# cmp-nct/ggllm.cpp

Hardware: NVIDIA B200
Metric: falcon40b_q4_k_decode_tokens_per_s (higher is better)
Workload: dtype int8 x int4 block dots (dp4a), fp32 accumulate; f32 KV/attention

## Files before the change

### ggllm.cpp_b200/csrc/common.cuh

```cuda
#pragma once
#include <cuda_runtime.h>
#include <cuda_fp16.h>
#include <cstdint>
#include <cstdio>
#include <cstdlib>

#define B200_CUDA_CHECK(expr)                                                                        \
    do {                                                                                             \
        cudaError_t err_ = (expr);                                                                   \
        if (err_ != cudaSuccess) {                                                                   \
            fprintf(stderr, "b200: CUDA error %d (%s) at %s:%d: %s\n", (int) err_,                   \
                    cudaGetErrorString(err_), __FILE__, __LINE__, #expr);                            \
            exit(1);                                                                                 \
        }                                                                                            \
    } while (0)

#define B200_ASSERT(x)                                                                               \
    do {                                                                                             \
        if (!(x)) {                                                                                  \
            fprintf(stderr, "B200_ASSERT: %s:%d: %s\n", __FILE__, __LINE__, #x);                     \
            abort();                                                                                 \
        }                                                                                            \
    } while (0)

enum : int {
    T_F32 = 0, T_F16 = 1, T_Q4_0 = 2, T_Q4_1 = 3, T_Q5_0 = 6, T_Q5_1 = 7, T_Q8_0 = 8, T_Q8_1 = 9,
    T_Q2_K = 10, T_Q3_K = 11, T_Q4_K = 12, T_Q5_K = 13, T_Q6_K = 14, T_Q8_K = 15,
};

static inline size_t round_up(size_t v, size_t a) { return (v + a - 1) / a * a; }

#define B200_CARVEOUT 25

#ifdef __CUDACC__

__device__ __forceinline__ uint4 ldg_stream_v4(const void * p) {
    uint4 r;
    asm volatile("ld.global.nc.L1::no_allocate.v4.u32 {%0,%1,%2,%3}, [%4];"
                 : "=r"(r.x), "=r"(r.y), "=r"(r.z), "=r"(r.w) : "l"(p));
    return r;
}
__device__ __forceinline__ uint2 ldg_stream_v2(const void * p) {
    uint2 r;
    asm volatile("ld.global.nc.L1::no_allocate.v2.u32 {%0,%1}, [%2];" : "=r"(r.x), "=r"(r.y) : "l"(p));
    return r;
}
__device__ __forceinline__ uint32_t ldg_stream_u32(const void * p) {
    uint32_t r;
    asm volatile("ld.global.nc.L1::no_allocate.u32 %0, [%1];" : "=r"(r) : "l"(p));
    return r;
}
__device__ __forceinline__ uint4 ldg_v4(const void * p) { return __ldg(reinterpret_cast<const uint4 *>(p)); }
__device__ __forceinline__ uint32_t ldg_u32(const void * p) { return __ldg(reinterpret_cast<const uint32_t *>(p)); }
__device__ __forceinline__ uint16_t ldg_u16(const void * p) { return __ldg(reinterpret_cast<const uint16_t *>(p)); }

__device__ __forceinline__ float f16_bits_to_f32(uint16_t h) { return __half2float(__ushort_as_half(h)); }
__device__ __forceinline__ uint16_t f32_to_f16_bits(float f) { return __half_as_ushort(__float2half_rn(f)); }

__device__ __forceinline__ float warp_sum(float v) {
#pragma unroll
    for (int o = 16; o > 0; o >>= 1) v += __shfl_xor_sync(0xffffffffu, v, o);
    return v;
}
__device__ __forceinline__ float warp_max(float v) {
#pragma unroll
    for (int o = 16; o > 0; o >>= 1) v = fmaxf(v, __shfl_xor_sync(0xffffffffu, v, o));
    return v;
}
__device__ __forceinline__ double warp_sum_d(double v) {
#pragma unroll
    for (int o = 16; o > 0; o >>= 1) v += __shfl_xor_sync(0xffffffffu, v, o);
    return v;
}

__device__ __forceinline__ int dp4a_ss(int a, int b, int c) { return __dp4a(a, b, c); }
__device__ __forceinline__ int dp4a_us(unsigned a, int b, int c) {
    int d;
    asm("dp4a.u32.s32 %0, %1, %2, %3;" : "=r"(d) : "r"(a), "r"(b), "r"(c));
    return d;
}

__device__ __forceinline__ uint32_t smem_u32(const void * p) { return (uint32_t) __cvta_generic_to_shared(p); }
__device__ __forceinline__ void mbar_init(uint64_t * bar, uint32_t count) {
    asm volatile("mbarrier.init.shared::cta.b64 [%0], %1;" :: "r"(smem_u32(bar)), "r"(count));
}
__device__ __forceinline__ void mbar_fence_init() { asm volatile("fence.mbarrier_init.release.cluster;" ::: "memory"); }
__device__ __forceinline__ void mbar_expect_tx(uint64_t * bar, uint32_t bytes) {
    asm volatile("mbarrier.arrive.expect_tx.shared::cta.b64 _, [%0], %1;" :: "r"(smem_u32(bar)), "r"(bytes) : "memory");
}
__device__ __forceinline__ void mbar_wait(uint64_t * bar, uint32_t phase) {
    asm volatile(
        "{\n\t.reg .pred p;\n\t"
        "WAIT_%=:\n\t"
        "mbarrier.try_wait.parity.shared::cta.b64 p, [%0], %1;\n\t"
        "@p bra DONE_%=;\n\t"
        "bra WAIT_%=;\n\t"
        "DONE_%=:\n\t}"
        :: "r"(smem_u32(bar)), "r"(phase) : "memory");
}
__device__ __forceinline__ void tma_load_1d(void * smem_dst, const void * gmem_src, uint32_t bytes, uint64_t * bar) {
    asm volatile("cp.async.bulk.shared::cluster.global.mbarrier::complete_tx::bytes [%0], [%1], %2, [%3];"
                 :: "r"(smem_u32(smem_dst)), "l"(gmem_src), "r"(bytes), "r"(smem_u32(bar)) : "memory");
}

__device__ __forceinline__ unsigned long long gtimer() { unsigned long long t; asm volatile("mov.u64 %0, %globaltimer;" : "=l"(t)); return t; }
__device__ __forceinline__ void trace_begin(unsigned long long * slot) { if (slot && threadIdx.x == 0) atomicMin(slot, gtimer()); }
__device__ __forceinline__ void trace_end(unsigned long long * slot) { if (slot && threadIdx.x == 0) atomicMax(slot + 1, gtimer()); }

#endif

unsigned long long * b200_trace_slot(const char * name);
```

### ggllm.cpp_b200/csrc/mmv_fast.cu

```cuda
#include "kernels.h"

#include "mmv_fast.cuh"

template <int TYPE, int NT, int J, int D, int MODE>
__device__ __forceinline__ void mmv_body(const WPlanes & W, const FastX & X, float * __restrict__ y, int64_t y_stride, const Epi & epi,
                                         const int cta, const int nctas, const int n, uint8_t * smem) {
    using T = FX<TYPE>;
    constexpr int NW = NT / 32;
    uint64_t * bar = reinterpret_cast<uint64_t *>(smem);
    float * partial = reinterpret_cast<float *>(smem + 16);
    double * red = reinterpret_cast<double *>(smem + 16 + 2 * NW * 4 * 4);
    int8_t * xq = reinterpret_cast<int8_t *>(smem + ((16 + 2 * NW * 4 * 4 + NW * 8 + 15) & ~15));
    const int tid = threadIdx.x, lane = tid & 31, warp = tid >> 5;
    const int P = W.nb * T::PPB;
    const ActQ & A = X.A;

    trace_begin(epi.trace);
    if (tid == 0 && MODE == 0) { mbar_init(bar, 1); mbar_fence_init(); }
    const int per = W.M / nctas, rem = W.M % nctas;
    const int row0 = cta * per + min(cta, rem), row1 = row0 + per + (cta < rem ? 1 : 0);
    const int nrows = row1 - row0;

    int gidx[J]; bool valid[J];
    WP wp[J];
    int aux[J];
#pragma unroll
    for (int j = 0; j < J; j++) { const int g = j * NT + tid; valid[j] = g < P; gidx[j] = valid[j] ? g : P - 1; wp[j] = T::wp(W, gidx[j]); aux[j] = piece_aux<TYPE>(gidx[j]); }

    typename T::WR w[D][J];
    ring_fill<TYPE, J, D>(w, wp, row0, row1);
    const L2PF pf = l2pf_of(W, X.l2_dist);
    if (pf.dist > 0 && tid == 0) l2_prefetch_rows(pf, min(row0 + D, row1), min(row0 + D + pf.dist, row1));

    if (!epi.late_wait) asm volatile("griddepcontrol.wait;" ::: "memory");
    typename T::XR xr[J];
    if (MODE == 0) {
        if (tid == 0) {
            mbar_expect_tx(bar, (uint32_t) W.K);
            tma_load_1d(xq, A.q + (size_t) n * W.K, (uint32_t) W.K, bar);
        }
        __syncthreads();
        mbar_wait(bar, 0);
#pragma unroll
        for (int j = 0; j < J; j++) xr[j] = valid[j] ? T::load_x(xq, A, n, gidx[j]) : zero_xr<TYPE>();
    } else if constexpr (T::HAS_PROLOGUE_QUANT) {
        const float * xrow = X.x + (size_t) n * X.x_stride;
        float mean = 0.f, scale = 1.f;
#pragma unroll
        for (int j = 0; j < J; j++) {
            int ea, eb; T::seg(gidx[j], ea, eb);
            float v[32];
#pragma unroll
            for (int i = 0; i < 4; i++) {
                const float4 a = *reinterpret_cast<const float4 *>(xrow + ea + 4 * i), b = *reinterpret_cast<const float4 *>(xrow + eb + 4 * i);
                v[4 * i] = a.x; v[4 * i + 1] = a.y; v[4 * i + 2] = a.z; v[4 * i + 3] = a.w;
                v[16 + 4 * i] = b.x; v[17 + 4 * i] = b.y; v[18 + 4 * i] = b.z; v[19 + 4 * i] = b.w;
            }
            if (MODE == 2 && J == 1) {
                if (X.ra) {
                    const float * ra = X.ra + (size_t) n * X.x_stride, * rb = X.rb + (size_t) n * X.x_stride;
#pragma unroll
                    for (int i = 0; i < 16; i++) { v[i] = __fadd_rn(__fadd_rn(ra[ea + i], rb[ea + i]), v[i]); v[16 + i] = __fadd_rn(__fadd_rn(ra[eb + i], rb[eb + i]), v[16 + i]); }
                }
                if (X.x_out && cta == 0 && valid[j]) {
                    float * xo = X.x_out + (size_t) n * X.x_stride;
#pragma unroll
                    for (int i = 0; i < 16; i++) { xo[ea + i] = v[i]; xo[eb + i] = v[16 + i]; }
                }
                double s = 0.0;
                if (valid[j]) {
#pragma unroll
                    for (int i = 0; i < 32; i++) s += (double) v[i];
                }
                s = warp_sum_d(s);
                if (lane == 0) red[warp] = s;
                __syncthreads();
                double t = 0.0;
#pragma unroll
                for (int wi = 0; wi < NW; wi++) t += red[wi];
                mean = (float) (t / W.K);
                __syncthreads();
                double s2 = 0.0;
                if (valid[j]) {
#pragma unroll
                    for (int i = 0; i < 32; i++) { const float c = __fsub_rn(v[i], mean); s2 += (double) __fmul_rn(c, c); }
                }
                s2 = warp_sum_d(s2);
                if (lane == 0) red[warp] = s2;
                __syncthreads();
                t = 0.0;
#pragma unroll
                for (int wi = 0; wi < NW; wi++) t += red[wi];
                scale = __fdiv_rn(1.0f, __fsqrt_rn(__fadd_rn((float) (t / W.K), 1e-5f)));
#pragma unroll
                for (int i = 0; i < 16; i++) {
                    v[i] = __fadd_rn(__fmul_rn(__fmul_rn(__fsub_rn(v[i], mean), scale), X.gamma[ea + i]), X.beta[ea + i]);
                    v[16 + i] = __fadd_rn(__fmul_rn(__fmul_rn(__fsub_rn(v[16 + i], mean), scale), X.gamma[eb + i]), X.beta[eb + i]);
                }
            }
            if (!valid[j]) {
#pragma unroll
                for (int i = 0; i < 32; i++) v[i] = 0.f;
            }
            xr[j] = T::quant_x(v, gidx[j], lane);
        }
        __syncthreads();
    }

    int gcount = 0;
    const int ekind = epi.kind; const float * r1p = epi.r1, * r2p = epi.r2;
    ring_run<TYPE, NT, J, D, false>(w, wp, row0, row1, wp, 0, 0, xr, aux, partial, gcount, 0, tid,
        [&](int row, float v) {
            if (ekind == EPI_GELU) v = gelu_lut(v);
            else if (ekind == EPI_ADD2) v = (v + r1p[(size_t) n * y_stride + row]) + r2p[(size_t) n * y_stride + row];
            y[(size_t) n * y_stride + row] = v;
        },
        [&]() { asm volatile("griddepcontrol.launch_dependents;" ::: "memory"); }, pf);
    if (epi.late_wait) asm volatile("griddepcontrol.wait;" ::: "memory");
    if (epi.qctr) {
        __shared__ int s_do;
        __threadfence();
        __syncthreads();
        if (nrows > 0) {
            for (int b = row0 >> 8; b <= (row1 - 1) >> 8; b++) {
                if (tid == 0) {
                    const unsigned cnt = (unsigned) (min(row1, (b + 1) << 8) - max(row0, b << 8));
                    const unsigned old = atomicAdd(epi.qctr + b, cnt);
                    s_do = old + cnt == 256u;
                    if (s_do) epi.qctr[b] = 0;
                }
                __syncthreads();
                if (s_do && warp == 0) {
                    __threadfence();
                    const float * src = y + (size_t) n * y_stride + (b << 8) + lane * 8;
                    const float4 p = __ldcg(reinterpret_cast<const float4 *>(src)), q = __ldcg(reinterpret_cast<const float4 *>(src) + 1);
                    const float v[8] = { p.x, p.y, p.z, p.w, q.x, q.y, q.z, q.w };
                    if (epi.qA.type == T_Q8_K) quantize_chunk8<T_Q8_K>(v, lane, epi.qA, n, (b << 8) + lane * 8);
                    else quantize_chunk8<T_Q8_0>(v, lane, epi.qA, n, (b << 8) + lane * 8);
                }
                __syncthreads();
            }
        }
    }
    trace_end(epi.trace);
}

template <int TYPE, int NT, int J, int D, int MODE>
__global__ void __launch_bounds__(NT) __maxnreg__(NT <= 256 ? 96 : 128) mmv_fast_kernel(const WPlanes W, const FastX X, float * __restrict__ y, int64_t y_stride, const Epi epi) {
    extern __shared__ __align__(16) uint8_t smem[];
    mmv_body<TYPE, NT, J, D, MODE>(W, X, y, y_stride, epi, (int) blockIdx.x, (int) gridDim.x, (int) blockIdx.y, smem);
}

static int fast_num_sms() {
    static int n = 0;
    if (!n) { int dev; B200_CUDA_CHECK(cudaGetDevice(&dev)); B200_CUDA_CHECK(cudaDeviceGetAttribute(&n, cudaDevAttrMultiProcessorCount, dev)); }
    return n;
}

template <int TYPE, int NT, int J, int D, int MODE>
static void launch_mode(const WPlanes & W, const FastX & X, float * y, int64_t y_stride, Epi epi, cudaStream_t stream) {
    const size_t smem = ((16 + 2 * (NT / 32) * 4 * 4 + (NT / 32) * 8 + 15) & ~15) + (size_t) ((W.K + 15) & ~15);
    static bool set = false;
    if (!set) { B200_CUDA_CHECK(cudaFuncSetAttribute(mmv_fast_kernel<TYPE, NT, J, D, MODE>, cudaFuncAttributeMaxDynamicSharedMemorySize, 100 * 1024));
        B200_CUDA_CHECK(cudaFuncSetAttribute(mmv_fast_kernel<TYPE, NT, J, D, MODE>, cudaFuncAttributePreferredSharedMemoryCarveout, B200_CARVEOUT)); set = true; }
    int ctas = fast_num_sms() * (NT == 128 ? 4 : NT == 160 || NT == 192 ? 3 : NT == 256 ? 2 : 1);
    if (ctas > (W.M + 3) / 4) ctas = (W.M + 3) / 4;
    cudaLaunchConfig_t cfg{};
    cfg.gridDim = dim3((unsigned) ctas, (unsigned) X.N); cfg.blockDim = dim3(NT); cfg.dynamicSmemBytes = smem; cfg.stream = stream;
    cudaLaunchAttribute attr[1];
    attr[0].id = cudaLaunchAttributeProgrammaticStreamSerialization;
    attr[0].val.programmaticStreamSerializationAllowed = 1;
    cfg.attrs = attr; cfg.numAttrs = getenv("B200_NO_PDL") ? 0 : 1;
    B200_CUDA_CHECK(cudaLaunchKernelEx(&cfg, mmv_fast_kernel<TYPE, NT, J, D, MODE>, W, X, y, y_stride, epi));
}
template <int TYPE, int NT, int J, int D>
static void launch_cfg(const WPlanes & W, const FastX & X, float * y, int64_t y_stride, Epi epi, cudaStream_t stream) {
    if (X.mode == 0) launch_mode<TYPE, NT, J, D, 0>(W, X, y, y_stride, epi, stream);
    else if constexpr (FX<TYPE>::HAS_PROLOGUE_QUANT) {
        if (X.mode == 1) launch_mode<TYPE, NT, J, D, 1>(W, X, y, y_stride, epi, stream);
        else if (J == 1) launch_mode<TYPE, NT, J, D, J == 1 ? 2 : 1>(W, X, y, y_stride, epi, stream);
        else B200_ASSERT(!"mmv_fast: LayerNorm prologue needs J == 1");
    } else B200_ASSERT(!"mmv_fast: this weight type takes quantised activations only (mode 0)");
}

template <int TYPE>
static bool launch_type(const WPlanes & W, const FastX & X, float * y, int64_t y_stride, Epi epi, cudaStream_t stream) {
    const int P = W.nb * FX<TYPE>::PPB;
    if (W.K > 64 * 1024) return false;
    if (X.mode == 2 && P > 512) return false;
    constexpr int D1 = FX<TYPE>::D256;
    if (P <= 128 && D1 == 4) launch_cfg<TYPE, 128, 1, D1>(W, X, y, y_stride, epi, stream);
    else if (P > 128 && P <= 160 && D1 == 8 && !getenv("B200_NO_NT160")) launch_cfg<TYPE, 160, 1, D1>(W, X, y, y_stride, epi, stream);
    else if (P <= 256) launch_cfg<TYPE, 256, 1, D1>(W, X, y, y_stride, epi, stream);
    else if (P > 256 && P <= 512 && D1 == 8 && X.mode == 0 && !getenv("B200_NO_NT256J2")) launch_cfg<TYPE, 256, 2, D1 / 2>(W, X, y, y_stride, epi, stream);
    else if (P <= 512) launch_cfg<TYPE, 512, 1, D1>(W, X, y, y_stride, epi, stream);
    else if (P > 512 && P <= 576 && D1 == 8 && X.mode == 0 && !getenv("B200_NO_NT192")) launch_cfg<TYPE, 192, 3, 2>(W, X, y, y_stride, epi, stream);
    else if (P <= 1024) launch_cfg<TYPE, 512, 2, D1 / 2>(W, X, y, y_stride, epi, stream);
    else if (P <= 2048 && D1 == 8) launch_cfg<TYPE, 512, 4, 2>(W, X, y, y_stride, epi, stream);
    else return false;
    return true;
}

bool launch_mmv_fast_x(const WPlanes & W, const FastX & X, float * y, int64_t y_stride, MmvEpilogue e, cudaStream_t stream) {
    const char * nm = W.M > 40000 ? "mmv_lmhead" : W.K > 16384 ? "mmv_down" : W.M > 16384 ? "mmv_up" : W.M > 8192 ? "mmv_qkv" : "mmv_wo";
    Epi epi = { e.kind, e.r1, e.r2, b200_trace_slot(nm), ActQ{}, nullptr, getenv("B200_NO_LATE_WAIT") ? 0 : e.late_wait };
    if (e.qout && e.qctr) {
        B200_ASSERT(X.N == 1 && W.M % 256 == 0 && e.qout->K == W.M && (e.qout->type == T_Q8_K || e.qout->type == T_Q8_0));
        epi.qA = *e.qout; epi.qctr = e.qctr;
    }
    static int dist_bytes = -1;
    if (dist_bytes < 0) { const char * s = getenv("B200_L2PF_KB"); dist_bytes = (s ? atoi(s) : 0) * 1024; }
    FastX Xp = X;
    Xp.l2_dist = W.stride[0] ? (int) (dist_bytes / W.stride[0]) : 0;
    switch (W.type) {
        case T_Q4_K: return launch_type<T_Q4_K>(W, Xp, y, y_stride, epi, stream);
        case T_Q4_0: return launch_type<T_Q4_0>(W, Xp, y, y_stride, epi, stream);
        case T_Q3_K: return X.mode == 0 && !getenv("B200_Q3K_GENERIC") && launch_type<T_Q3_K>(W, Xp, y, y_stride, epi, stream);
    }
    return false;
}
bool mmv_fast_supports(int wtype, int K, int mode) {
    if (wtype != T_Q4_K && wtype != T_Q4_0) return false;
    const int P = wtype == T_Q4_K ? K / 32 : K / 32;
    return K <= 64 * 1024 && P <= (mode == 2 ? 512 : 2048);
}
bool mmv_fast_fills_sm(const WPlanes & W) {
    if ((W.type != T_Q4_K && W.type != T_Q4_0) || getenv("B200_NO_NT192")) return false;
    const int P = W.K / 32;
    return P > 512 && P <= 576;
}
bool launch_mmv_fast(const WPlanes & W, const ActQ & A, float * y, int64_t y_stride, MmvEpilogue e, cudaStream_t stream) {
    FastX X{}; X.mode = 0; X.A = A; X.N = A.N;
    return launch_mmv_fast_x(W, X, y, y_stride, e, stream);
}
```

### ggllm.cpp_b200/csrc/mmv_fast.cuh

```cuda
#pragma once
#include "kernels.h"
#include "actquant.cuh"

struct Epi { int kind; const float * r1; const float * r2; unsigned long long * trace; ActQ qA; unsigned * qctr; int late_wait; };


__device__ __forceinline__ int dot16(const uint32_t w0, const uint32_t w1, const uint32_t w2, const uint32_t w3, const uint4 x) {
    int s = dp4a_us(w0, (int) x.x, 0); s = dp4a_us(w1, (int) x.y, s); s = dp4a_us(w2, (int) x.z, s); return dp4a_us(w3, (int) x.w, s);
}
__device__ __forceinline__ int dp2a_lo_su(int pair16, uint32_t bytes) { int d; asm("dp2a.lo.s32.u32 %0, %1, %2, %3;" : "=r"(d) : "r"(pair16), "r"(bytes), "r"(0)); return d; }
__device__ __forceinline__ int dp2a_hi_su(int pair16, uint32_t bytes) { int d; asm("dp2a.hi.s32.u32 %0, %1, %2, %3;" : "=r"(d) : "r"(pair16), "r"(bytes), "r"(0)); return d; }
__device__ __forceinline__ int dp2a_lo_ss(int pair16, uint32_t bytes, int c) { int d; asm("dp2a.lo.s32.s32 %0, %1, %2, %3;" : "=r"(d) : "r"(pair16), "r"(bytes), "r"(c)); return d; }
__device__ __forceinline__ int dp2a_hi_ss(int pair16, uint32_t bytes, int c) { int d; asm("dp2a.hi.s32.s32 %0, %1, %2, %3;" : "=r"(d) : "r"(pair16), "r"(bytes), "r"(c)); return d; }
__device__ __forceinline__ float gelu_lut(float v) {
    const float f = __half2float(__float2half_rn(v));
    const float g = 0.5f * f * (1.0f + tanhf(0.79788456080286535587989211986876f * f * (1.0f + 0.044715f * f * f)));
    return __half2float(__float2half_rn(g));
}

struct WP { const uint8_t * b0, * b1, * b2, * b3; uint32_t s0, s1, s2, s3; };
__device__ __forceinline__ const uint8_t * opaque_ptr(const uint8_t * p) { unsigned long long v = (unsigned long long) p; asm volatile("" : "+l"(v)); return (const uint8_t *) v; }

template <int TYPE> struct FX;

template <> struct FX<T_Q4_K> {
    static constexpr int PPB = 8;
    static constexpr bool HAS_PROLOGUE_QUANT = true;
    static constexpr int D256 = 8;
    struct XR { uint4 xl, xh; int bs; float xd; };
    struct WR { uint4 q; uint32_t sm, dd; };
    __device__ static XR load_x(const int8_t * xq, const ActQ & A, int n, int g) {
        const int b = g >> 3, pc = g & 7, p = pc >> 1, half = pc & 1;
        XR r;
        const int e0 = b * 256 + 64 * p + 16 * half;
        r.xl = *reinterpret_cast<const uint4 *>(xq + e0);
        r.xh = *reinterpret_cast<const uint4 *>(xq + e0 + 32);
        const int16_t * bs = A.bs + (size_t) n * (A.K / 16) + b * 16 + 4 * p + half;
        r.bs = ((int) bs[0] & 0xffff) | ((int) bs[2] << 16);
        r.xd = A.d[(size_t) n * (A.K / 256) + b];
        return r;
    }
    __device__ static void seg(int g, int & ea, int & eb) { const int b = g >> 3, pc = g & 7; ea = b * 256 + 64 * (pc >> 1) + 16 * (pc & 1); eb = ea + 32; }
    __device__ static XR quant_x(const float (&v)[32], int g, int lane) {
        int ea, eb; seg(g, ea, eb);
        float amax = 0.f, vmax = 0.f; int imax = 0;
#pragma unroll
        for (int i = 0; i < 32; i++) { const float ax = fabsf(v[i]); const int idx = (i < 16 ? ea : eb - 16) + i; if (ax > amax || (ax == amax && ax > 0.f && idx < imax)) { amax = ax; vmax = v[i]; imax = idx; } }
#pragma unroll
        for (int o = 1; o < 8; o <<= 1) {
            const float oa = __shfl_xor_sync(0xffffffffu, amax, o), ov = __shfl_xor_sync(0xffffffffu, vmax, o);
            const int oi = __shfl_xor_sync(0xffffffffu, imax, o);
            if (oa > amax || (oa == amax && oi < imax)) { amax = oa; vmax = ov; imax = oi; }
        }
        XR r;
        const bool zero = amax == 0.f;
        const float iscale = zero ? 0.f : __fdiv_rn(-128.f, vmax);
        r.xd = zero ? 0.f : __fdiv_rn(1.f, iscale);
        int s0 = 0, s1 = 0;
        uint32_t w[8];
#pragma unroll
        for (int i = 0; i < 8; i++) {
            uint32_t pk = 0;
#pragma unroll
            for (int k = 0; k < 4; k++) {
                const int q = zero ? 0 : min(127, __float2int_rn(__fmul_rn(iscale, v[4 * i + k])));
                if (i < 4) s0 += q; else s1 += q;
                pk |= (uint32_t) (q & 0xff) << (8 * k);
            }
            w[i] = pk;
        }
        r.xl = make_uint4(w[0], w[1], w[2], w[3]); r.xh = make_uint4(w[4], w[5], w[6], w[7]);
        r.bs = (s0 & 0xffff) | (s1 << 16);
        (void) lane;
        return r;
    }
    __device__ static WP wp(const WPlanes & W, int g) {
        WP r; r.b0 = opaque_ptr(W.p[0] + (size_t) g * 16); r.b1 = opaque_ptr(W.p[1] + (size_t) (g >> 1) * 4); r.b2 = opaque_ptr(W.p[2] + (size_t) (g >> 3) * 4);
        r.s0 = W.stride[0]; r.s1 = W.stride[1]; r.s2 = W.stride[2];
        return r;
    }
    __device__ static WR load_w(const WP & p, uint32_t row) {
        WR r;
        r.q = ldg_stream_v4(p.b0 + (uint64_t) row * p.s0);
        r.sm = ldg_u32(p.b1 + (uint64_t) row * p.s1);
        r.dd = ldg_u32(p.b2 + (uint64_t) row * p.s2);
        return r;
    }
    __device__ static float dot(const WR & w, const XR & x) {
        const int il = dot16(w.q.x & 0x0F0F0F0F, w.q.y & 0x0F0F0F0F, w.q.z & 0x0F0F0F0F, w.q.w & 0x0F0F0F0F, x.xl);
        const int ih = dot16(w.q.x & 0xF0F0F0F0, w.q.y & 0xF0F0F0F0, w.q.z & 0xF0F0F0F0, w.q.w & 0xF0F0F0F0, x.xh) >> 4;
        const int isum = dp2a_lo_su((il & 0xffff) | (ih << 16), w.sm);
        const int msum = dp2a_hi_su(x.bs, w.sm);
        const float2 dm = __half22float2(*reinterpret_cast<const __half2 *>(&w.dd));
        return (dm.x * x.xd) * (float) isum - (dm.y * x.xd) * (float) msum;
    }
};

template <> struct FX<T_Q4_0> {
    static constexpr int PPB = 1;
    static constexpr bool HAS_PROLOGUE_QUANT = true;
    static constexpr int D256 = 8;
    struct XR { uint4 xl, xh; int bs; float xd; };
    struct WR { uint4 q; uint32_t d; };
    __device__ static XR load_x(const int8_t * xq, const ActQ & A, int n, int g) {
        XR r;
        r.xl = *reinterpret_cast<const uint4 *>(xq + g * 32);
        r.xh = *reinterpret_cast<const uint4 *>(xq + g * 32 + 16);
        r.bs = A.bs[(size_t) n * (A.K / 32) + g];
        r.xd = A.d[(size_t) n * (A.K / 32) + g];
        return r;
    }
    __device__ static void seg(int g, int & ea, int & eb) { ea = g * 32; eb = ea + 16; }
    __device__ static XR quant_x(const float (&v)[32], int, int) {
        float amax = 0.f;
#pragma unroll
        for (int i = 0; i < 32; i++) amax = fmaxf(amax, fabsf(v[i]));
        const float id = amax != 0.f ? __fdiv_rn(127.f, amax) : 0.f;
        XR r;
        r.xd = __half2float(__float2half_rn(__fdiv_rn(amax, 127.f)));
        int s = 0;
        uint32_t w[8];
#pragma unroll
        for (int i = 0; i < 8; i++) {
            uint32_t pk = 0;
#pragma unroll
            for (int k = 0; k < 4; k++) { const int q = __float2int_rn(__fmul_rn(v[4 * i + k], id)); s += q; pk |= (uint32_t) (q & 0xff) << (8 * k); }
            w[i] = pk;
        }
        r.xl = make_uint4(w[0], w[1], w[2], w[3]); r.xh = make_uint4(w[4], w[5], w[6], w[7]);
        r.bs = s;
        return r;
    }
    __device__ static WP wp(const WPlanes & W, int g) {
        WP r; r.b0 = opaque_ptr(W.p[0] + (size_t) g * 16); r.b1 = opaque_ptr(W.p[1] + (size_t) g * 2); r.b2 = nullptr;
        r.s0 = W.stride[0]; r.s1 = W.stride[1]; r.s2 = 0;
        return r;
    }
    __device__ static WR load_w(const WP & p, uint32_t row) {
        WR r;
        r.q = ldg_stream_v4(p.b0 + (uint64_t) row * p.s0);
        r.d = ldg_u16(p.b1 + (uint64_t) row * p.s1);
        return r;
    }
    __device__ static float dot(const WR & w, const XR & x) {
        int s = dot16(w.q.x & 0x0F0F0F0F, w.q.y & 0x0F0F0F0F, w.q.z & 0x0F0F0F0F, w.q.w & 0x0F0F0F0F, x.xl);
        s += dot16(w.q.x & 0xF0F0F0F0, w.q.y & 0xF0F0F0F0, w.q.z & 0xF0F0F0F0, w.q.w & 0xF0F0F0F0, x.xh) >> 4;
        s -= 8 * x.bs;
        return ((float) s * f16_bits_to_f32((uint16_t) w.d)) * x.xd;
    }
};

template <> struct FX<T_Q3_K> {
    static constexpr int PPB = 4;
    static constexpr bool HAS_PROLOGUE_QUANT = false;
    static constexpr int D256 = 4;
    struct XR { uint4 x[4]; int bsA, bsB; float xd; };
    struct WR { uint4 q, hm; uint32_t sc, d; };
    __device__ static XR load_x(const int8_t * xq, const ActQ & A, int n, int g) {
        const int b = g >> 2, pc = g & 3, hn = pc >> 1, c = pc & 1;
        XR r;
        const int16_t * bs = A.bs + (size_t) n * (A.K / 16) + b * 16 + 8 * hn + c;
#pragma unroll
        for (int quad = 0; quad < 4; quad++) r.x[quad] = *reinterpret_cast<const uint4 *>(xq + b * 256 + 128 * hn + 32 * quad + 16 * c);
        r.bsA = ((int) bs[0] & 0xffff) | ((int) bs[2] << 16);
        r.bsB = ((int) bs[4] & 0xffff) | ((int) bs[6] << 16);
        r.xd = A.d[(size_t) n * (A.K / 256) + b];
        return r;
    }
    __device__ static void seg(int, int & ea, int & eb) { ea = 0; eb = 0; }
    __device__ static XR quant_x(const float (&)[32], int, int) { return XR{}; }
    __device__ static WP wp(const WPlanes & W, int g) {
        WP r;
        r.b0 = opaque_ptr(W.p[0] + (size_t) g * 16); r.b1 = opaque_ptr(W.p[1] + (size_t) (g >> 2) * 32 + (g & 1) * 16);
        r.b2 = opaque_ptr(W.p[2] + (size_t) g * 4);  r.b3 = opaque_ptr(W.p[3] + (size_t) (g >> 2) * 2);
        r.s0 = W.stride[0]; r.s1 = W.stride[1]; r.s2 = W.stride[2]; r.s3 = W.stride[3];
        return r;
    }
    __device__ static WR load_w(const WP & p, uint32_t row) {
        WR r;
        r.q = ldg_stream_v4(p.b0 + (uint64_t) row * p.s0);
        r.hm = ldg_v4(p.b1 + (uint64_t) row * p.s1);
        r.sc = ldg_u32(p.b2 + (uint64_t) row * p.s2);
        r.d = ldg_u16(p.b3 + (uint64_t) row * p.s3);
        return r;
    }
    __device__ static float dot(const WR & w, const XR & x, int hsh) {
        const uint32_t q[4] = { w.q.x, w.q.y, w.q.z, w.q.w }, hm[4] = { w.hm.x, w.hm.y, w.hm.z, w.hm.w };
        const uint32_t hbase = 0x01010101u << hsh;
        int i[4];
#pragma unroll
        for (int quad = 0; quad < 4; quad++) {
            const uint32_t qm = 0x03030303u << (2 * quad), hmk = hbase << quad;
            const int dq = dot16(q[0] & qm, q[1] & qm, q[2] & qm, q[3] & qm, x.x[quad]);
            const int dh = dot16(hm[0] & hmk, hm[1] & hmk, hm[2] & hmk, hm[3] & hmk, x.x[quad]);
            i[quad] = (dq >> (2 * quad)) + ((dh >> (hsh + quad)) << 2);
        }
        int isum = dp2a_lo_ss((i[0] & 0xffff) | (i[1] << 16), w.sc, 0);
        isum = dp2a_hi_ss((i[2] & 0xffff) | (i[3] << 16), w.sc, isum);
        int bsum = dp2a_lo_ss(x.bsA, w.sc, 0);
        bsum = dp2a_hi_ss(x.bsB, w.sc, bsum);
        return (f16_bits_to_f32((uint16_t) w.d) * x.xd) * (float) (isum - 4 * bsum);
    }
};

template <int G> __device__ __forceinline__ float transpose_reduce(const float (&acc)[G], int lane, int & row_of_lane) {
    float w;
    if (G == 4) {
        const bool hi = lane & 16;
        float v0 = hi ? acc[2] : acc[0], v1 = hi ? acc[3] : acc[1];
        v0 += __shfl_xor_sync(0xffffffffu, hi ? acc[0] : acc[2], 16);
        v1 += __shfl_xor_sync(0xffffffffu, hi ? acc[1] : acc[3], 16);
        const bool mid = lane & 8;
        w = mid ? v1 : v0;
        w += __shfl_xor_sync(0xffffffffu, mid ? v0 : v1, 8);
        w += __shfl_xor_sync(0xffffffffu, w, 4);
        row_of_lane = (hi ? 2 : 0) + (mid ? 1 : 0);
    } else if (G == 2) {
        const bool hi = lane & 16;
        w = hi ? acc[G - 1] : acc[0];
        w += __shfl_xor_sync(0xffffffffu, hi ? acc[0] : acc[G - 1], 16);
        w += __shfl_xor_sync(0xffffffffu, w, 8);
        w += __shfl_xor_sync(0xffffffffu, w, 4);
        row_of_lane = hi ? 1 : 0;
    } else {
        w = acc[0];
        w += __shfl_xor_sync(0xffffffffu, w, 16);
        w += __shfl_xor_sync(0xffffffffu, w, 8);
        w += __shfl_xor_sync(0xffffffffu, w, 4);
        row_of_lane = 0;
    }
    w += __shfl_xor_sync(0xffffffffu, w, 2);
    w += __shfl_xor_sync(0xffffffffu, w, 1);
    return w;
}


struct L2PF { const uint8_t * p[3]; uint32_t s[3]; int dist; };
__device__ __forceinline__ void l2_prefetch_rows(const L2PF & pf, int a, int b) {
    if (b <= a) return;
#pragma unroll
    for (int i = 0; i < 3; i++) {
        if (!pf.p[i]) continue;
        const uint8_t * src = pf.p[i] + (size_t) a * pf.s[i];
        const uint32_t bytes = (uint32_t) (b - a) * pf.s[i];
        asm volatile("cp.async.bulk.prefetch.L2.global [%0], %1;" :: "l"(src), "r"(bytes) : "memory");
    }
}
__device__ __forceinline__ L2PF l2pf_of(const WPlanes & W, int dist) {
    L2PF r; r.dist = dist;
#pragma unroll
    for (int i = 0; i < 3; i++) { r.p[i] = W.p[i]; r.s[i] = W.stride[i]; }
    return r;
}

__device__ __forceinline__ void named_sync(int id, int n) { asm volatile("bar.sync %0, %1;" :: "r"(id), "r"(n) : "memory"); }

template <int TYPE> __device__ __forceinline__ int piece_aux(int g) { return TYPE == T_Q3_K ? 4 * ((g & 3) >> 1) : 0; }
template <int TYPE> __device__ __forceinline__ float piece_dot(const typename FX<TYPE>::WR & w, const typename FX<TYPE>::XR & x, int aux) {
    if constexpr (TYPE == T_Q3_K) return FX<TYPE>::dot(w, x, aux); else return FX<TYPE>::dot(w, x);
}
template <int TYPE> __device__ __forceinline__ typename FX<TYPE>::XR zero_xr() {
    typename FX<TYPE>::XR r{}; return r;
}

template <int TYPE, int J, int D>
__device__ __forceinline__ void ring_fill(typename FX<TYPE>::WR (&w)[D][J], const WP (&wp)[J], int r0, int r1) {
    if (r1 <= r0) return;
#pragma unroll
    for (int s = 0; s < D; s++) {
        const uint32_t row = (uint32_t) min(r0 + s, r1 - 1);
#pragma unroll
        for (int j = 0; j < J; j++) w[s][j] = FX<TYPE>::load_w(wp[j], row);
    }
}

template <int TYPE, int NTG, int J, int D, bool CHECKED, bool HASNEXT, class Store>
__device__ __forceinline__ void ring_pass(typename FX<TYPE>::WR (&w)[D][J], const WP (&wp)[J], const int r0, const int nrows, const int npad, const int base,
                                          const WP (&wpn)[J], const int n0, const int n1,
                                          const typename FX<TYPE>::XR (&xr)[J], const int (&aux)[J], float * partial, int & gcount, const int bar_id, const int tg, Store & store) {
    using T = FX<TYPE>;
    constexpr int NWG = NTG / 32, G = (D % 4 == 0) ? 4 : (D % 2 == 0) ? 2 : 1;
    const int lane = tg & 31, warp = tg >> 5;
    float acc[G];
#pragma unroll
    for (int s = 0; s < D; s++) {
        float a = piece_dot<TYPE>(w[s][0], xr[0], aux[0]);
#pragma unroll
        for (int j = 1; j < J; j++) a += piece_dot<TYPE>(w[s][j], xr[j], aux[j]);
        acc[s % G] = a;
        const int nxt = base + D + s;
        if (!CHECKED || nxt < nrows) {
#pragma unroll
            for (int j = 0; j < J; j++) w[s][j] = T::load_w(wp[j], (uint32_t) (r0 + nxt));
        } else if (HASNEXT && nxt >= npad && n1 > n0) {
            const uint32_t k = (uint32_t) min(n0 + nxt - npad, n1 - 1);
#pragma unroll
            for (int j = 0; j < J; j++) w[s][j] = T::load_w(wpn[j], k);
        }
        if ((s % G) == G - 1) {
            const int gi = (base + s) / G;
            int rl;
            const float v0 = transpose_reduce<G>(acc, lane, rl);
            float * part = partial + (gcount & 1) * NWG * G;
            gcount++;
            if ((lane & (G == 4 ? 7 : G == 2 ? 15 : 31)) == 0) part[warp * G + rl] = v0;
            named_sync(bar_id, NTG);
            if (tg < G) {
                const int row = r0 + gi * G + tg;
                if (!CHECKED || row < r0 + nrows) {
                    float v = 0.f;
#pragma unroll
                    for (int wi = 0; wi < NWG; wi++) v += part[wi * G + tg];
                    store(row, v);
                }
            }
        }
    }
}

template <int TYPE, int NTG, int J, int D, bool HASNEXT, class Store, class Tail>
__device__ __forceinline__ void ring_run(typename FX<TYPE>::WR (&w)[D][J], const WP (&wp)[J], const int r0, const int r1,
                                         const WP (&wpn)[J], const int n0, const int n1,
                                         const typename FX<TYPE>::XR (&xr)[J], const int (&aux)[J], float * partial, int & gcount, const int bar_id, const int tg,
                                         Store store, Tail before_tail, const L2PF pf = L2PF{ { nullptr, nullptr, nullptr }, { 0, 0, 0 }, 0 }) {
    const int nrows = r1 - r0, npad = (nrows + D - 1) / D * D;
    if (npad == 0) { before_tail(); if (HASNEXT) ring_fill<TYPE, J, D>(w, wpn, n0, n1); return; }
    int base = 0;
    for (; base + 2 * D <= nrows; base += D) {
        if (pf.dist > 0 && tg == 0) l2_prefetch_rows(pf, min(r0 + base + D + pf.dist, r1), min(r0 + base + 2 * D + pf.dist, r1));
        ring_pass<TYPE, NTG, J, D, false, false>(w, wp, r0, nrows, npad, base, wpn, n0, n1, xr, aux, partial, gcount, bar_id, tg, store);
    }
    before_tail();
    for (; base < npad; base += D)
        ring_pass<TYPE, NTG, J, D, true, HASNEXT>(w, wp, r0, nrows, npad, base, wpn, n0, n1, xr, aux, partial, gcount, bar_id, tg, store);
}
```

Baseline: 210.2.

## Replace per-group CTA barrier with mbarrier reduction ring in matvec

Result: slower. 163.1, median of 6 (-22.4%).

```diff
diff --git a/ggllm.cpp_b200/csrc/common.cuh b/ggllm.cpp_b200/csrc/common.cuh
--- a/ggllm.cpp_b200/csrc/common.cuh
+++ b/ggllm.cpp_b200/csrc/common.cuh
@@ -81,9 +81,8 @@
 }
 
 __device__ __forceinline__ uint32_t smem_u32(const void * p) { return (uint32_t) __cvta_generic_to_shared(p); }
-__device__ __forceinline__ void mbar_init(uint64_t * bar, uint32_t count) {
-    asm volatile("mbarrier.init.shared::cta.b64 [%0], %1;" :: "r"(smem_u32(bar)), "r"(count));
-}
+__device__ __forceinline__ void mbar_init(uint32_t bar, uint32_t count) { asm volatile("mbarrier.init.shared::cta.b64 [%0], %1;" :: "r"(bar), "r"(count)); }
+__device__ __forceinline__ void mbar_init(uint64_t * bar, uint32_t count) { mbar_init(smem_u32(bar), count); }
 __device__ __forceinline__ void mbar_fence_init() { asm volatile("fence.mbarrier_init.release.cluster;" ::: "memory"); }
 __device__ __forceinline__ void mbar_expect_tx(uint64_t * bar, uint32_t bytes) {
     asm volatile("mbarrier.arrive.expect_tx.shared::cta.b64 _, [%0], %1;" :: "r"(smem_u32(bar)), "r"(bytes) : "memory");
diff --git a/ggllm.cpp_b200/csrc/mmv_fast.cu b/ggllm.cpp_b200/csrc/mmv_fast.cu
--- a/ggllm.cpp_b200/csrc/mmv_fast.cu
+++ b/ggllm.cpp_b200/csrc/mmv_fast.cu
@@ -1,22 +1,38 @@
 #include "kernels.h"
 
 #include "mmv_fast.cuh"
+
+template <int NT, int D> struct MmvSmem {
+    static constexpr int NW = NT / 32, G = ring_group<D>(), R = 4, LAG = 2;
+    using Ring = RedRing<NW, G, R>;
+    static constexpr int xbar = 0;
+    static constexpr int ring = 8;
+    static constexpr int red = (ring + Ring::BYTES + 7) & ~7;
+    static constexpr int xq = (red + NW * 8 + 15) & ~15;
+    static size_t bytes(int K) { return (size_t) xq + (size_t) ((K + 15) & ~15); }
+};
 
 template <int TYPE, int NT, int J, int D, int MODE>
 __device__ __forceinline__ void mmv_body(const WPlanes & W, const FastX & X, float * __restrict__ y, int64_t y_stride, const Epi & epi,
                                          const int cta, const int nctas, const int n, uint8_t * smem) {
     using T = FX<TYPE>;
+    using L = MmvSmem<NT, D>;
     constexpr int NW = NT / 32;
-    uint64_t * bar = reinterpret_cast<uint64_t *>(smem);
-    float * partial = reinterpret_cast<float *>(smem + 16);
-    double * red = reinterpret_cast<double *>(smem + 16 + 2 * NW * 4 * 4);
-    int8_t * xq = reinterpret_cast<int8_t *>(smem + ((16 + 2 * NW * 4 * 4 + NW * 8 + 15) & ~15));
+    uint64_t * bar = reinterpret_cast<uint64_t *>(smem + L::xbar);
+    const typename L::Ring rr = { smem_u32(smem + L::ring) };
+    double * red = reinterpret_cast<double *>(smem + L::red);
+    int8_t * xq = reinterpret_cast<int8_t *>(smem + L::xq);
     const int tid = threadIdx.x, lane = tid & 31, warp = tid >> 5;
     const int P = W.nb * T::PPB;
     const ActQ & A = X.A;
 
     trace_begin(epi.trace);
-    if (tid == 0 && MODE == 0) { mbar_init(bar, 1); mbar_fence_init(); }
+    if (tid == 0) {
+        if (MODE == 0) mbar_init(bar, 1);
+#pragma unroll
+        for (int s = 0; s < L::R; s++) { mbar_init(rr.full(s), NW * L::G); mbar_init(rr.empty(s), L::G); }
+        mbar_fence_init();
+    }
     const int per = W.M / nctas, rem = W.M % nctas;
     const int row0 = cta * per + min(cta, rem), row1 = row0 + per + (cta < rem ? 1 : 0);
     const int nrows = row1 - row0;
@@ -107,9 +123,8 @@
         __syncthreads();
     }
 
-    int gcount = 0;
     const int ekind = epi.kind; const float * r1p = epi.r1, * r2p = epi.r2;
-    ring_run<TYPE, NT, J, D, false>(w, wp, row0, row1, wp, 0, 0, xr, aux, partial, gcount, 0, tid,
+    ring_run<TYPE, NT, J, D, L::R, L::LAG>(w, wp, row0, row1, xr, aux, rr, tid,
         [&](int row, float v) {
             if (ekind == EPI_GELU) v = gelu_lut(v);
             else if (ekind == EPI_ADD2) v = (v + r1p[(size_t) n * y_stride + row]) + r2p[(size_t) n * y_stride + row];
@@ -159,7 +174,7 @@
 
 template <int TYPE, int NT, int J, int D, int MODE>
 static void launch_mode(const WPlanes & W, const FastX & X, float * y, int64_t y_stride, Epi epi, cudaStream_t stream) {
-    const size_t smem = ((16 + 2 * (NT / 32) * 4 * 4 + (NT / 32) * 8 + 15) & ~15) + (size_t) ((W.K + 15) & ~15);
+    const size_t smem = MmvSmem<NT, D>::bytes(W.K);
     static bool set = false;
     if (!set) { B200_CUDA_CHECK(cudaFuncSetAttribute(mmv_fast_kernel<TYPE, NT, J, D, MODE>, cudaFuncAttributeMaxDynamicSharedMemorySize, 100 * 1024));
         B200_CUDA_CHECK(cudaFuncSetAttribute(mmv_fast_kernel<TYPE, NT, J, D, MODE>, cudaFuncAttributePreferredSharedMemoryCarveout, B200_CARVEOUT)); set = true; }
diff --git a/ggllm.cpp_b200/csrc/mmv_fast.cuh b/ggllm.cpp_b200/csrc/mmv_fast.cuh
--- a/ggllm.cpp_b200/csrc/mmv_fast.cuh
+++ b/ggllm.cpp_b200/csrc/mmv_fast.cuh
@@ -253,8 +253,6 @@
     return r;
 }
 
-__device__ __forceinline__ void named_sync(int id, int n) { asm volatile("bar.sync %0, %1;" :: "r"(id), "r"(n) : "memory"); }
-
 template <int TYPE> __device__ __forceinline__ int piece_aux(int g) { return TYPE == T_Q3_K ? 4 * ((g & 3) >> 1) : 0; }
 template <int TYPE> __device__ __forceinline__ float piece_dot(const typename FX<TYPE>::WR & w, const typename FX<TYPE>::XR & x, int aux) {
     if constexpr (TYPE == T_Q3_K) return FX<TYPE>::dot(w, x, aux); else return FX<TYPE>::dot(w, x);
@@ -263,6 +261,38 @@
     typename FX<TYPE>::XR r{}; return r;
 }
 
+template <int D> constexpr int ring_group() { return (D % 4 == 0) ? 4 : (D % 2 == 0) ? 2 : 1; }
+
+template <int NW, int G, int R> struct RedRing {
+    uint32_t base;
+    __device__ uint32_t full(int slot) const { return base + 8 * slot; }
+    __device__ uint32_t empty(int slot) const { return base + 8 * (R + slot); }
+    __device__ uint32_t part(int slot, int wi, int r) const { return base + 16 * R + 4 * ((slot * NW + wi) * G + r); }
+    static constexpr int BYTES = 16 * R + 4 * R * NW * G;
+};
+__device__ __forceinline__ bool mbar_try_wait_u32(uint32_t bar, uint32_t phase) {
+    uint32_t ok;
+    asm volatile("{\n\t.reg .pred p;\n\tmbarrier.try_wait.parity.shared::cta.b64 p, [%1], %2;\n\tselp.u32 %0, 1, 0, p;\n\t}" : "=r"(ok) : "r"(bar), "r"(phase) : "memory");
+    return ok != 0;
+}
+__device__ __forceinline__ void mbar_wait_u32(uint32_t bar, uint32_t phase) { while (!mbar_try_wait_u32(bar, phase)) {} }
+__device__ __forceinline__ void mbar_arrive_u32(uint32_t bar) { asm volatile("mbarrier.arrive.shared::cta.b64 _, [%0];" :: "r"(bar) : "memory"); }
+__device__ __forceinline__ void sts_f32(uint32_t a, float v) { asm volatile("st.shared.f32 [%0], %1;" :: "r"(a), "f"(v) : "memory"); }
+__device__ __forceinline__ float lds_f32(uint32_t a) { float v; asm volatile("ld.shared.f32 %0, [%1];" : "=f"(v) : "r"(a) : "memory"); return v; }
+
+template <int NW, int G, int R, bool CHECKED, class Store>
+__device__ __forceinline__ void ring_reduce(const RedRing<NW, G, R> & red, const int gr, const int r0, const int nrows, const int warp, const int lane, Store & store) {
+    if (gr % NW != warp || lane >= G) return;
+    const int slot = gr % R;
+    mbar_wait_u32(red.full(slot), (uint32_t) ((gr / R) & 1));
+    float v = 0.f;
+#pragma unroll
+    for (int wi = 0; wi < NW; wi++) v += lds_f32(red.part(slot, wi, lane));
+    mbar_arrive_u32(red.empty(slot));
+    const int row = r0 + gr * G + lane;
+    if (!CHECKED || row < r0 + nrows) store(row, v);
+}
+
 template <int TYPE, int J, int D>
 __device__ __forceinline__ void ring_fill(typename FX<TYPE>::WR (&w)[D][J], const WP (&wp)[J], int r0, int r1) {
     if (r1 <= r0) return;
@@ -274,13 +304,12 @@
     }
 }
 
-template <int TYPE, int NTG, int J, int D, bool CHECKED, bool HASNEXT, class Store>
-__device__ __forceinline__ void ring_pass(typename FX<TYPE>::WR (&w)[D][J], const WP (&wp)[J], const int r0, const int nrows, const int npad, const int base,
-                                          const WP (&wpn)[J], const int n0, const int n1,
-                                          const typename FX<TYPE>::XR (&xr)[J], const int (&aux)[J], float * partial, int & gcount, const int bar_id, const int tg, Store & store) {
+template <int TYPE, int NT, int J, int D, int R, int LAG, bool CHECKED, class Store>
+__device__ __forceinline__ void ring_pass(typename FX<TYPE>::WR (&w)[D][J], const WP (&wp)[J], const int r0, const int nrows, const int base,
+                                          const typename FX<TYPE>::XR (&xr)[J], const int (&aux)[J], const RedRing<NT / 32, ring_group<D>(), R> & red, const int tid, Store & store) {
     using T = FX<TYPE>;
-    constexpr int NWG = NTG / 32, G = (D % 4 == 0) ? 4 : (D % 2 == 0) ? 2 : 1;
-    const int lane = tg & 31, warp = tg >> 5;
+    constexpr int NW = NT / 32, G = ring_group<D>();
+    const int lane = tid & 31, warp = tid >> 5;
     float acc[G];
 #pragma unroll
     for (int s = 0; s < D; s++) {
@@ -288,49 +317,43 @@
 #pragma unroll
         for (int j = 1; j < J; j++) a += piece_dot<TYPE>(w[s][j], xr[j], aux[j]);
         acc[s % G] = a;
+        if ((s % G) == G - 1) {
+            const int gi = base / G + s / G, slot = gi % R;
+            int rl;
+            const float v0 = transpose_reduce<G>(acc, lane, rl);
+            if ((lane & (G == 4 ? 7 : G == 2 ? 15 : 31)) == 0) {
+                if (gi >= R) mbar_wait_u32(red.empty(slot), (uint32_t) ((gi / R - 1) & 1));
+                sts_f32(red.part(slot, warp, rl), v0);
+                mbar_arrive_u32(red.full(slot));
+            }
+            if (gi >= LAG) ring_reduce<NW, G, R, CHECKED>(red, gi - LAG, r0, nrows, warp, lane, store);
+        }
         const int nxt = base + D + s;
         if (!CHECKED || nxt < nrows) {
 #pragma unroll
             for (int j = 0; j < J; j++) w[s][j] = T::load_w(wp[j], (uint32_t) (r0 + nxt));
-        } else if (HASNEXT && nxt >= npad && n1 > n0) {
-            const uint32_t k = (uint32_t) min(n0 + nxt - npad, n1 - 1);
-#pragma unroll
-            for (int j = 0; j < J; j++) w[s][j] = T::load_w(wpn[j], k);
-        }
-        if ((s % G) == G - 1) {
-            const int gi = (base + s) / G;
-            int rl;
-            const float v0 = transpose_reduce<G>(acc, lane, rl);
-            float * part = partial + (gcount & 1) * NWG * G;
-            gcount++;
-            if ((lane & (G == 4 ? 7 : G == 2 ? 15 : 31)) == 0) part[warp * G + rl] = v0;
-            named_sync(bar_id, NTG);
-            if (tg < G) {
-                const int row = r0 + gi * G + tg;
-                if (!CHECKED || row < r0 + nrows) {
-                    float v = 0.f;
-#pragma unroll
-                    for (int wi = 0; wi < NWG; wi++) v += part[wi * G + tg];
-                    store(row, v);
-                }
-            }
-        }
-    }
-}
-
-template <int TYPE, int NTG, int J, int D, bool HASNEXT, class Store, class Tail>
+        }
+    }
+}
+
+template <int TYPE, int NT, int J, int D, int R, int LAG, class Store, class Tail>
 __device__ __forceinline__ void ring_run(typename FX<TYPE>::WR (&w)[D][J], const WP (&wp)[J], const int r0, const int r1,
-                                         const WP (&wpn)[J], const int n0, const int n1,
-                                         const typename FX<TYPE>::XR (&xr)[J], const int (&aux)[J], float * partial, int & gcount, const int bar_id, const int tg,
+                                         const typename FX<TYPE>::XR (&xr)[J], const int (&aux)[J], const RedRing<NT / 32, ring_group<D>(), R> & red, const int tid,
                                          Store store, Tail before_tail, const L2PF pf = L2PF{ { nullptr, nullptr, nullptr }, { 0, 0, 0 }, 0 }) {
+    constexpr int G = ring_group<D>();
+    static_assert(LAG >= 0 && LAG < R, "the reduction ring deadlocks unless LAG < R");
     const int nrows = r1 - r0, npad = (nrows + D - 1) / D * D;
-    if (npad == 0) { before_tail(); if (HASNEXT) ring_fill<TYPE, J, D>(w, wpn, n0, n1); return; }
+    if (npad == 0) { before_tail(); return; }
     int base = 0;
     for (; base + 2 * D <= nrows; base += D) {
-        if (pf.dist > 0 && tg == 0) l2_prefetch_rows(pf, min(r0 + base + D + pf.dist, r1), min(r0 + base + 2 * D + pf.dist, r1));
-        ring_pass<TYPE, NTG, J, D, false, false>(w, wp, r0, nrows, npad, base, wpn, n0, n1, xr, aux, partial, gcount, bar_id, tg, store);
+        if (pf.dist > 0 && tid == 0) l2_prefetch_rows(pf, min(r0 + base + D + pf.dist, r1), min(r0 + base + 2 * D + pf.dist, r1));
+        ring_pass<TYPE, NT, J, D, R, LAG, false>(w, wp, r0, nrows, base, xr, aux, red, tid, store);
     }
     before_tail();
     for (; base < npad; base += D)
-        ring_pass<TYPE, NTG, J, D, true, HASNEXT>(w, wp, r0, nrows, npad, base, wpn, n0, n1, xr, aux, partial, gcount, bar_id, tg, store);
-}
+        ring_pass<TYPE, NT, J, D, R, LAG, true>(w, wp, r0, nrows, base, xr, aux, red, tid, store);
+    const int ng = npad / G;
+#pragma unroll
+    for (int k = LAG; k > 0; k--)
+        if (ng - k >= 0) ring_reduce<NT / 32, G, R, true>(red, ng - k, r0, nrows, tid >> 5, tid & 31, store);
+}
```
